# fakerlove1/HPFG

Hardware: AMD Instinct MI355X
Metric: labeled+unlabeled images/sec/node, U-Net 224x224 ACDC-shaped (Mean-Teacher step) (higher is better)
Workload: dtype bf16x3 (fp32 storage; products as split-bf16 MFMA hi*hi+hi*lo+lo*hi, fp32 accumulate); 1 GPU; mean_teacher_unet_224x224 (BASELINE configs[1]): U-Net 1ch->4cls, 8 labelled + 8 unlabelled per GPU, student fwd+bwd + train-mode teacher fwd + CE/Dice/MSE + SGD + EMA; size=224, hipgraph=True, sync_bn=False, parallelism=dp1, math=bf16x3

## Files before the change

hpfg_amd/_lib.py:

```python
from __future__ import annotations

import ctypes as C
import os
import threading

_HERE = os.path.dirname(os.path.abspath(__file__))
LIB_PATH = os.path.join(_HERE, "lib", "libhpfg_hip.so")

BN_MEAN, BN_RSTD, BN_SCALE, BN_SHIFT, BN_K1, BN_K2, BN_K3, BN_SPARE, BN_ROWS = range(9)
ACT_NONE, ACT_PLAIN, ACT_STRIDED, ACT_BNACT, ACT_BNACT_POOL, ACT_UP2X, ACT_DZ, ACT_SPLIT16, ACT_UPBWD = range(9)
OPT_CONV_THIN, OPT_FIRST_MFMA, OPT_FIRST_WGRAD, OPT_NARROW_DEEP = 0, 1, 2, 3
LOSS_NSUM = 32
LOSS_MAX_CLASSES = 16
ACC_MAX_SHARDS = 8
VERSION = 136
RESIZE_TAPS = 36
MATH_F32, MATH_BF16X3 = 0, 1


class HipLibraryError(RuntimeError):
    pass


class Act(C.Structure):
    _fields_ = [("z", C.c_void_p), ("bn", C.c_void_p), ("aux", C.c_void_p), ("mode", C.c_int32), ("C", C.c_int32),
                ("Hs", C.c_int32), ("Ws", C.c_int32), ("pstride", C.c_int32), ("aux_pstride", C.c_int32),
                ("bn_stride", C.c_int32), ("bn_coff", C.c_int32), ("sn", C.c_int32), ("sc", C.c_int32), ("sy", C.c_int32),
                ("sx", C.c_int32), ("drop_p", C.c_float), ("drop_seed", C.c_uint32), ("drop_mask", C.c_void_p), ("seed_dev", C.c_void_p),
                ("bn_acc", C.c_void_p), ("bn_gamma", C.c_void_p), ("bn_beta", C.c_void_p), ("bn_count", C.c_float), ("bn_eps", C.c_float),
                ("bn_shards", C.c_int32), ("reserved1", C.c_int32)]


class ConvArgs(C.Structure):
    _fields_ = [("a0", Act), ("a1", Act), ("wpk", C.c_void_p), ("bias", C.c_void_p), ("out", C.c_void_p),
                ("stat_partials", C.c_void_p), ("out_pstride", C.c_int32), ("Cout", C.c_int32), ("CoutPad", C.c_int32),
                ("N", C.c_int32), ("H", C.c_int32), ("W", C.c_int32), ("taps", C.c_int32), ("math", C.c_int32),
                ("bwd_stats", C.c_int32), ("bwd_of", Act), ("out2", C.c_void_p), ("out_split", C.c_int32), ("out2_pstride", C.c_int32),
                ("stat_acc", C.c_void_p), ("stat_shards", C.c_int32), ("reserved2", C.c_int32), ("stage_out", C.c_void_p), ("side_sums", C.c_void_p)]


class WgradArgs(C.Structure):
    _fields_ = [("a0", Act), ("a1", Act), ("g", Act), ("slab", C.c_void_p), ("dw_oihw", C.c_void_p), ("Cin", C.c_int32),
                ("CinPad", C.c_int32), ("Cout", C.c_int32), ("CoutPad", C.c_int32), ("N", C.c_int32), ("H", C.c_int32),
                ("W", C.c_int32), ("taps", C.c_int32), ("S", C.c_int32), ("math", C.c_int32), ("defer_reduce", C.c_int32)]


class PeerX(C.Structure):
    _fields_ = [("mbox", C.c_void_p * 8), ("epoch", C.c_void_p), ("err", C.c_void_p), ("world", C.c_int32), ("rank", C.c_int32),
                ("slot", C.c_int32), ("cap", C.c_int32), ("slot_bytes", C.c_int64)]


class PeerBuf(C.Structure):
    _fields_ = [("win", C.c_void_p * 8), ("epoch", C.c_void_p), ("err", C.c_void_p), ("world", C.c_int32), ("rank", C.c_int32),
                ("slice", C.c_int64), ("n", C.c_int64), ("stride", C.c_int64)]


class FusedBwdArgs(C.Structure):
    _fields_ = [("d", ConvArgs), ("xa0", Act), ("xa1", Act), ("slab", C.c_void_p), ("Cin", C.c_int32), ("CinPad", C.c_int32),
                ("Cout", C.c_int32), ("CoutPad", C.c_int32)]


class AugSample(C.Structure):
    _fields_ = [("img_off", C.c_int64), ("lab_off", C.c_int64), ("h", C.c_int32), ("w", C.c_int32), ("mode", C.c_int32), ("k", C.c_int32),
                ("axis", C.c_int32), ("tab_off", C.c_int32), ("m00", C.c_double), ("m01", C.c_double), ("m10", C.c_double),
                ("m11", C.c_double), ("off_y", C.c_double), ("off_x", C.c_double)]


class BnAccDesc(C.Structure):
    _fields_ = [("acc", C.c_void_p), ("gamma", C.c_void_p), ("beta", C.c_void_p), ("running_mean", C.c_void_p), ("running_var", C.c_void_p),
                ("bn", C.c_void_p), ("C", C.c_int32), ("count", C.c_float), ("shards", C.c_int32), ("reserved", C.c_int32)]


class BnAccBwdDesc(C.Structure):
    _fields_ = [("acc", C.c_void_p), ("gamma", C.c_void_p), ("bn", C.c_void_p), ("dgamma", C.c_void_p), ("dbeta", C.c_void_p),
                ("C", C.c_int32), ("count", C.c_float), ("shards", C.c_int32), ("reserved", C.c_int32)]


class SlabDesc(C.Structure):
    _fields_ = [("slab", C.c_void_p), ("dw_oihw", C.c_void_p), ("S", C.c_int32), ("taps", C.c_int32), ("Cin", C.c_int32),
                ("CinPad", C.c_int32), ("Cout", C.c_int32), ("CoutPad", C.c_int32)]


class PackDesc(C.Structure):
    _fields_ = [("w_oihw", C.c_void_p), ("b", C.c_void_p), ("wpk_fwd", C.c_void_p), ("wpk_dgrad", C.c_void_p),
                ("bias_pad", C.c_void_p), ("wpk16_fwd", C.c_void_p), ("wpk16_dgrad", C.c_void_p), ("Cout", C.c_int32), ("Cin", C.c_int32),
                ("CoutPad", C.c_int32), ("CinPad", C.c_int32), ("taps", C.c_int32), ("kc", C.c_int32)]


class LossArgs(C.Structure):
    _fields_ = [("logits", C.c_void_p), ("t_logits", C.c_void_p), ("labels0", C.c_void_p), ("labels1", C.c_void_p),
                ("coef", C.c_void_p), ("partials", C.c_void_p), ("sums", C.c_void_p), ("out", C.c_void_p),
                ("dlogits", C.c_void_p), ("N", C.c_int32), ("n_lab", C.c_int32), ("H", C.c_int32), ("W", C.c_int32),
                ("C", C.c_int32), ("world", C.c_int32), ("input_is_prob", C.c_int32), ("teacher_is_prob", C.c_int32),
                ("t_unlab_only", C.c_int32), ("reserved0", C.c_int32), ("cons_mask", C.c_void_p)]


class PredBlocks(C.Structure):
    _fields_ = [("p", C.c_void_p * 8), ("n_blocks", C.c_int32), ("per_block", C.c_int32)]
# ... 75 lines not shown
    "hpfg_linear_wgrad": (_i, [_p, _p, _p, _p, _l, _i, _i, _p]),
    "hpfg_linear_wgrad_splits": (_i, [_l, _i, _i]),
    "hpfg_tok_col_stats": (_i, [_p, _l, _i, _p, _p, _p]),
    "hpfg_tok_stat_blocks": (_i, [_l]),
    "hpfg_bnrelu_apply": (_i, [_p, _p, _p, _p, _p, _p, _f, _l, _p, _l, _i, _p]),
    "hpfg_bnrelu_bwd": (_i, [_p, _p, _p, _p, _p, _p, _p, _f, _l, _p, _p, _p, _l, _i, _p]),
    "hpfg_noise_add": (_i, [_p, _p, _p, _l, _l, _f, _f, _f, _p]),
    "hpfg_uncertainty_mask": (_i, [C.POINTER(PredBlocks), _i, _i, _i, _i, _i, _p, _p, _p, _p]),
    "hpfg_mix_samples": (_i, [_p, _p, _p, _p, _i, _l, _p]),
    "hpfg_softmax_mix": (_i, [_p, _p, _p, _p, _i, _i, _i, _i, _p]),
    "hpfg_pool_scatter_add": (_i, [C.POINTER(Act), _p, _i, _p, _i, _i, _i, _i, _p]),
    "hpfg_upsample2x_bwd": (_i, [_p, _i, _p, _i, _i, _i, _i, _p]),
    "hpfg_upsample2x_bwd_sums": (_i, [_p, _i, _p, _i, _i, _i, _i, _p, _p]),
    "hpfg_upsample2x_bwd_blocks": (_i, [_i, _i, _i, _i]),
    "hpfg_loss_blocks": (_i, [_i, _i, _i]),
    "hpfg_loss_nsum": (_i, [_i]),
    "hpfg_seg_loss_partials": (_i, [C.POINTER(LossArgs), _p]),
    "hpfg_seg_loss_finalize": (_i, [C.POINTER(LossArgs), _p]),
    "hpfg_seg_loss_bwd": (_i, [C.POINTER(LossArgs), _p, _p]),
    "hpfg_argmax_labels": (_i, [_p, _i, _i, _i, _i, _p, _p, _p, _p]),
    "hpfg_cutmix_blend": (_i, [_p, _p, _p, _p, _l, _p]),
    "hpfg_sgd_step": (_i, [_p, _p, _p, _l, _p, _f, _f, _f, _p]),
    "hpfg_adamw_step": (_i, [_p, _p, _p, _p, _l, _p, _p, _f, _f, _f, _f, _f, _p]),
    "hpfg_ema_update": (_i, [_p, _p, _l, _p, _p]),
    "hpfg_sgd_ema_step": (_i, [_p, _p, _p, _l, _p, _f, _f, _f, _p, _l, _p, _p]),
    "hpfg_attn_mfma_fwd": (_i, [_p, _p, _p, _i, _i, _i, _i, _f, _p]),
    "hpfg_attn_mfma_bwd": (_i, [_p, _p, _p, _p, _p, _p, _i, _i, _i, _i, _f, _p]),
    "hpfg_attn_mfma_blocks": (_i, [_i]),
    "hpfg_attn_mfma_fwd_hd": (_i, [_p, _p, _p, _i, _i, _i, _i, _i, _f, _p]),
    "hpfg_attn_mfma_bwd_hd": (_i, [_p, _p, _p, _p, _p, _p, _i, _i, _i, _i, _i, _f, _p]),
    "hpfg_attn_mfma_scratch_floats": (_l, [_i, _i, _i, _i]),
    "hpfg_attn_keys_max": (_i, []),
    "hpfg_attn_keys_fwd": (_i, [_p, _p, _p, _p, _i, _i, _i, _i, _i, _f, _i, _p]),
    "hpfg_attn_keys_bwd": (_i, [_p, _p, _p, _p, _p, _p, _p, _p, _i, _i, _i, _i, _i, _f, _i, _p]),
    "hpfg_attn_keys_scratch_floats": (_l, [_i, _i, _i, _i, _i, _i]),
    "hpfg_attn_fwd_hd": (_i, [_p, _p, _p, _i, _i, _i, _i, _i, _f, _p]),
    "hpfg_attn_bwd_hd": (_i, [_p, _p, _p, _p, _p, _p, _i, _i, _i, _i, _i, _f, _p]),
    "hpfg_gemm_f32": (_i, [_p, _l, _l, _p, _l, _l, _p, _l, _i, _i, _i, _p, _i, _i, _p]),
    "hpfg_gemm_f32_splitk": (_i, [_p, _l, _l, _p, _l, _l, _p, _l, _i, _i, _i, _p, _i, _i, _p, _p]),
    "hpfg_gemm_f32_splits": (_i, [_i, _i, _i]),
    "hpfg_gemm_bf16x3": (_i, [_p, _l, _l, _p, _l, _l, _p, _l, _i, _i, _i, _p, _i, _i, _p]),
    "hpfg_gemm_bf16x3_splits": (_i, [_i, _i, _i]),
    "hpfg_gemm_bf16x3_splitk": (_i, [_p, _l, _l, _p, _l, _l, _p, _l, _i, _i, _i, _p, _i, _i, _p, _p]),
    "hpfg_gemm_bf16x3_ok": (_i, [_p, _l, _l, _p, _l, _l, _i, _i, _i]),
    "hpfg_gemm_tn_bf16x3": (_i, [_p, _p, _p, _p, _l, _i, _i, _i, _p]),
    "hpfg_gemm_tn_splits": (_i, [_l, _i, _i]),
    "hpfg_col_sum2": (_i, [_p, _l, _i, _l, _p, _p, _p]),
    "hpfg_col_sum_splits": (_i, [_l]),
    "hpfg_col_sum": (_i, [_p, _l, _i, _l, _p, _p]),
    "hpfg_relu_bwd": (_i, [_p, _p, _l, _p]),
    "hpfg_neck_pool_fwd": (_i, [_p, _i, _i, _i, _i, _i, _i, _p, _p, _p]),
    "hpfg_neck_pool_bwd": (_i, [_p, _p, _i, _i, _i, _i, _i, _p, _p]),
    "hpfg_l2norm_fwd": (_i, [_p, _i, _i, _i, _i, _i, _p, _p, _p]),
    "hpfg_l2norm_bwd": (_i, [_p, _p, _p, _i, _i, _i, _i, _i, _p, _p, _p]),
    "hpfg_ntxent_rows": (_i, [_p, _i, _f, _p, _p, _p]),
}

_lock = threading.Lock()
_lib = None


def load() -> C.CDLL:
    global _lib
    if _lib is not None:
        return _lib
    with _lock:
        if _lib is not None:
            return _lib
        if not os.path.exists(LIB_PATH):
            raise HipLibraryError(
                f"{LIB_PATH} not found: build it with `python -c 'import __graft_entry__ as g; g.build()'` "
                f"or `make -C hpfg_amd/csrc`. There is no CPU fallback for the HIP path.")
        lib = C.CDLL(LIB_PATH)
        for name, (res, args) in PROTOTYPES.items():
            fn = getattr(lib, name)
            fn.restype = res
            fn.argtypes = args
        if lib.hpfg_version() != VERSION:
            raise HipLibraryError(f"libhpfg_hip.so version {lib.hpfg_version()} != binding version {VERSION}; rebuild")
        if os.environ.get("HPFG_FIRST_WGRAD", "1") == "0":
            lib.hpfg_set_option(OPT_FIRST_WGRAD, 0)
        if os.environ.get("HPFG_NARROW_DEEP") is not None:
            lib.hpfg_set_option(OPT_NARROW_DEEP, int(os.environ["HPFG_NARROW_DEEP"]))
        _lib = lib
    return _lib


def check(rc: int, what: str):
    if rc != 0:
        msg = load().hpfg_last_error().decode("utf-8", "replace")
        raise HipLibraryError(f"{what} failed (rc={rc}): {msg}")


def ptr(t):
    return None if t is None else t.data_ptr()


def none_act() -> Act:
    return Act()
```

hpfg_amd/csrc/conv_bf16_kernel.h:

```cpp
#pragma once
#include <stdlib.h>
#include "stage.h"

namespace hpfg_conv16 {

using namespace hpfg_stage;

template <int TH_, int TW_, int WM_, int WN_, int NI_, int TAPS_, int KC_>
struct Cfg {
  static constexpr int TH = TH_, TW = TW_, WM = WM_, WN = WN_, NI = NI_, TAPS = TAPS_, KC = KC_;
  static constexpr int MI = TH * TW / 16 / WM;
  static constexpr int BN = 16 * NI * WN;
  static constexpr int HALO = TAPS == 9 ? 1 : 0;
  static constexpr int HP = TH + 2 * HALO, WP = TW + 2 * HALO;
  static constexpr int RS = TW == 16 ? WP : (TAPS == 9 ? 24 : 8);
  static constexpr int NSLOT = (HP * RS + 15) / 16 * 16;
  static constexpr int NG = KC / 8;
  static constexpr int PLANE = NSLOT * 16;
  static constexpr int BUF_BYTES = NG * 2 * PLANE;
  static constexpr int KSTEPS = TAPS == 1 ? 1 : (KC == 32 ? 9 : 5);
  static constexpr int NPIECE = HP * WP * NG;
  static constexpr int NLD = (NPIECE + 255) / 256;
  static_assert(WM * WN == 4, "4 waves per workgroup");
  static_assert(256 % NG == 0, "a thread must keep one channel group");
// ... 93 lines not shown
    for (int m = 0; m < C::MI; ++m) {
      const int pxl = (wm * C::MI + m) * 16 + (lane & 15);
      const int gy = ty0 + pxl / C::TW, gx = tx0 + pxl % C::TW;
      if (pool) {
        if (gy < H && gx < W && co < p.Cout) {
          const f32x4 v = acc[m][j];
          float* dA = const_cast<float*>(p.bwd_of.aux);
          const long p00 = ((long)n * p.bwd_of.Hs + 2 * gy) * p.bwd_of.Ws + 2 * gx;
          f32x4 z4[4], g4[4];
#pragma unroll
          for (int k = 0; k < 4; ++k) {
            const long off = p00 + (k >> 1) * p.bwd_of.Ws + (k & 1);
            z4[k] = *reinterpret_cast<const f32x4*>(p.bwd_of.z + off * p.bwd_of.pstride + co);
            g4[k] = *reinterpret_cast<const f32x4*>(dA + off * p.bwd_of.aux_pstride + co);
          }
#pragma unroll
          for (int r = 0; r < 4; ++r) {
            float y[4];
#pragma unroll
            for (int k = 0; k < 4; ++k) y[k] = z4[k][r] * tsc[r] + tsh[r];
            float best = lrelu(y[0]);
            int bi = 0;
#pragma unroll
            for (int k = 1; k < 4; ++k) {
              const float a = lrelu(y[k]);
              if (a > best) {
                best = a;
                bi = k;
              }
            }
#pragma unroll
            for (int k = 0; k < 4; ++k) {
              g4[k][r] += bi == k ? v[r] : 0.f;
              const float gg = y[k] > 0.f ? g4[k][r] : HPFG_LEAKY * g4[k][r];
              s1[j][r] += gg;
              s2[j][r] += gg * z4[k][r];
            }
          }
#pragma unroll
          for (int k = 0; k < 4; ++k) {
            const long off = p00 + (k >> 1) * p.bwd_of.Ws + (k & 1);
            *reinterpret_cast<f32x4*>(dA + off * p.bwd_of.aux_pstride + co) = g4[k];
          }
        }
        continue;
      }
      if (gy < H && gx < W && co < p.Cout) {
        f32x4 v = acc[m][j] + b;
        float* o = (p.out_split && co >= p.out_split) ? p.out2 + ((n * H + gy) * W + gx) * p.out2_pstride + (co - p.out_split)
                                                       : p.out + ((n * H + gy) * W + gx) * p.out_pstride + co;
        if (p.math & 0x100) {
        } else if (vec) {
          *reinterpret_cast<f32x4*>(o) = v;
        } else {
#pragma unroll
          for (int r = 0; r < 4; ++r) {
            if (co + r < p.Cout) o[r] = v[r];
            else v[r] = 0.f;
          }
        }
        if (bwd) {
          const long pix = ((long)n * H + gy) * W + gx;
          const f32x4 z = zq[m];
          uint32_t km = 0xFu;
          if (p.bwd_of.drop_p > 0.f) km = keep4(p.bwd_of, bcx, (uint32_t)(pix * p.bwd_of.C + co));
#pragma unroll
          for (int r = 0; r < 4; ++r) {
            float gg = (km >> r) & 1u ? v[r] * bcx.inv_keep : 0.f;
            gg = z[r] * tsc[r] + tsh[r] > 0.f ? gg : HPFG_LEAKY * gg;
            s1[j][r] += gg;
            s2[j][r] += gg * z[r];
          }
        } else {
          s1[j] += v;
          s2[j] += v * v;
        }
      }
    }
  }
}

template <class C, int BWD = 0>
__device__ __forceinline__ void conv16_flush_stats(const HpfgConvArgs& p, f32x4 (&s1)[C::NI], f32x4 (&s2)[C::NI], float* ldsf, int tid, int lane, int wm,
                                                   int wn, int cb, int row) {
  if ((!p.stat_partials && !p.stat_acc) || (p.math & 0x1000)) return;
#pragma unroll
  for (int j = 0; j < C::NI; ++j)
#pragma unroll
    for (int r = 0; r < 4; ++r) {
      float a = s1[j][r], b = s2[j][r];
#pragma unroll
      for (int o = 1; o < 16; o <<= 1) {
        a += __shfl_xor(a, o);
        b += __shfl_xor(b, o);
      }
      s1[j][r] = a;
      s2[j][r] = b;
    }
  if ((lane & 15) == 0) {
#pragma unroll
    for (int j = 0; j < C::NI; ++j) {
      const int cl = (wn * C::NI + j) * 16 + (lane >> 4) * 4;
      *reinterpret_cast<f32x4*>(ldsf + (0 * C::WM + wm) * C::BN + cl) = s1[j];
      *reinterpret_cast<f32x4*>(ldsf + (1 * C::WM + wm) * C::BN + cl) = s2[j];
    }
  }
  __syncthreads();
  if (tid < 2 * C::BN) {
    const int which = tid / C::BN, cl = tid % C::BN;
    float t = 0.f;
#pragma unroll
    for (int w = 0; w < C::WM; ++w) t += ldsf[(which * C::WM + w) * C::BN + cl];
    const int co = cb * C::BN + cl;
    if (BWD && p.bwd_stats && which == 1 && co < p.Cout) {
      float sg = 0.f;
#pragma unroll
      for (int w = 0; w < C::WM; ++w) sg += ldsf[w * C::BN + cl];
      const float* tb = p.bwd_of.bn + p.bwd_of.bn_coff + co;
      t = tb[HPFG_BN_RSTD * p.bwd_of.bn_stride] * (t - tb[HPFG_BN_MEAN * p.bwd_of.bn_stride] * sg);
    }
    if (p.stat_acc && co < p.Cout)
      hpfg_acc_add(p.stat_acc, p.CoutPad, ((int)blockIdx.z * (int)gridDim.y + (int)blockIdx.y) * (int)gridDim.x + (int)blockIdx.x & (p.stat_shards - 1), which, co, t);
    if (p.stat_partials && co < p.CoutPad) p.stat_partials[((long)row * 2 + which) * p.CoutPad + co] = t;
  }
}

#define HPFG16_MFMA3(ACC, AH, AL, BH, BL)                              \
  ACC = __builtin_amdgcn_mfma_f32_16x16x32_bf16(BH, AH, ACC, 0, 0, 0); \
  ACC = __builtin_amdgcn_mfma_f32_16x16x32_bf16(BL, AH, ACC, 0, 0, 0); \
  ACC = __builtin_amdgcn_mfma_f32_16x16x32_bf16(BH, AL, ACC, 0, 0, 0);

template <class C>
struct UpGeo {
  static constexpr int SH = C::TH / 2 + 3, SW = C::TW / 2 + 3;
  static constexpr int NPIECE = SH * SW * C::NG;
  static constexpr int BYTES = SH * SW * C::KC * 4;
  static_assert(NPIECE <= 256, "one source piece per thread");
};
template <int KIND>
constexpr int eff_nr() { return KIND == HPFG_KIND_CAT ? 2 : RawCount<KIND>::N; }

__device__ __forceinline__ int up_base(int o0, int L) {
  const float r = L > 1 ? (float)(L - 1) / (float)(2 * L - 1) : 0.f;
  return (int)(r * (float)(o0 < 0 ? 0 : o0));
}

template <class C, int KIND>
constexpr int wg_per_cu() {
  return (C::KSTEPS == 5 && C::NI == 1 && RawCount<KIND>::N <= 2) ? 3 : 2;
}

#ifdef HPFG_TRACE
#define HPFG_TR(ID)                                                                                        \
  if (tr_on && tr_i < 255) {                                                                               \
    tr_buf[tr_i++] = ((unsigned long long)(ID) << 56) | (__builtin_amdgcn_s_memtime() & 0xffffffffffffffull); \
  }
#define HPFG_TR_REAL(ID)                                                                                   \
  if (tr_on && tr_i < 255) {                                                                               \
    tr_buf[tr_i++] = ((unsigned long long)(ID) << 56) | (__builtin_amdgcn_s_memrealtime() & 0xffffffffffffffull); \
  }
#else
#define HPFG_TR(ID)
#define HPFG_TR_REAL(ID)
#endif

template <class C, int KIND, int BWD = 0>
__global__ __launch_bounds__(256, (wg_per_cu<C, KIND>())) void conv_bf16x3_kernel(HpfgConvArgs p, int tiles_x, int tiles_y) {
  static_assert(C::TAPS == 9, "persistent kernel is the 3x3 path");
  constexpr int STAT_BYTES = 2 * 4 * C::BN * 4;
  constexpr int NR = eff_nr<KIND>();
  constexpr bool CATK = KIND == HPFG_KIND_CAT;
  constexpr int UP_BYTES = CATK ? UpGeo<C>::BYTES : 0;
  __shared__ __attribute__((aligned(16))) unsigned char lds[2 * C::BUF_BYTES + STAT_BYTES + UP_BYTES];
  float* ldsf = reinterpret_cast<float*>(lds + 2 * C::BUF_BYTES);
  float* ldsU = reinterpret_cast<float*>(lds + 2 * C::BUF_BYTES + STAT_BYTES);
  (void)ldsU;
  constexpr bool TABK = tab_in_lds<KIND>();
  __shared__ __attribute__((aligned(16))) float ldsBN[TABK ? tab_rows<KIND>() * HPFG_BN_CMAX : 4];
  (void)ldsBN;
  const int tid = threadIdx.x, lane = tid & 63, wave = tid >> 6;
  const int wm = wave % C::WM, wn = wave / C::WM;
  const int cb = blockIdx.y;
  const int H = p.H, W = p.W;
  const int ntiles = tiles_x * tiles_y, nwork = ntiles * p.N;
  const ActCtx cx0 = make_ctx(p.a0);
  constexpr bool SIDE = KIND != HPFG_KIND_PLAIN && C::TH == 4;
  const bool dzw = SIDE && p.stage_out != nullptr && cb == 0;
  (void)dzw;
#ifdef HPFG_TRACE
  const bool tr_on = (p.math & 0x2000) && tid == 0;
  unsigned long long* tr_buf = reinterpret_cast<unsigned long long*>(p.stat_partials) + 256 * ((long)blockIdx.y * gridDim.x + blockIdx.x);
  int tr_i = 0;
#endif
  HPFG_TR_REAL(11)
  HPFG_TR(1)

  f32x4 acc[C::MI][C::NI];
#pragma unroll
  for (int m = 0; m < C::MI; ++m)
#pragma unroll
    for (int j = 0; j < C::NI; ++j) acc[m][j] = f32x4{0.f, 0.f, 0.f, 0.f};

  const int kg = lane >> 4;
  const int gl = C::KC == 32 ? kg : (kg & 1);
  int aoff[C::MI];
// ... 348 lines not shown
        f32x4 v[2] = {f32x4{0.f, 0.f, 0.f, 0.f}, f32x4{0.f, 0.f, 0.f, 0.f}};
#pragma unroll
        for (int hq = 0; hq < 2; ++hq) {
          f32x4 t[HPFG_UPB_TAPS][HPFG_UPB_TAPS];
#pragma unroll
          for (int a = 0; a < HPFG_UPB_TAPS; ++a) {
            const float* row = src + (long)upI[q.ly][a] * Wo * ps + 4 * hq;
#pragma unroll
            for (int b = 0; b < HPFG_UPB_TAPS; ++b) t[a][b] = *reinterpret_cast<const f32x4*>(row + ix[b]);
          }
          f32x4 acc = {0.f, 0.f, 0.f, 0.f};
#pragma unroll
          for (int a = 0; a < HPFG_UPB_TAPS; ++a) {
            f32x4 h = wx[0] * t[a][0];
#pragma unroll
            for (int b = 1; b < HPFG_UPB_TAPS; ++b) h += wx[b] * t[a][b];
            acc += hpfg_own_vgpr(upW[q.ly][a]) * h;
          }
#pragma unroll
          for (int j = 0; j < 4; ++j) v[hq][j] = ok ? acc[j] : 0.f;
        }
        store_piece<C, HPFG_KIND_PLAIN>(lds, q, v[0], v[1]);
        if (side && ok) {
          if (p.stage_out) {
            float* d = p.stage_out + ((long)(n * H + gy) * W + gx) * p.a0.C + c0c;
            *reinterpret_cast<f32x4*>(d) = v[0];
            *reinterpret_cast<f32x4*>(d + 4) = v[1];
          }
          cs0 += v[0];
          cs1 += v[1];
        }
      }
      if (side && p.side_sums) {
        *reinterpret_cast<f32x4*>(upS + tid * 8) = cs0;
        *reinterpret_cast<f32x4*>(upS + tid * 8 + 4) = cs1;
      }
    } else {
#pragma unroll
    for (int i = 0; i < C::NLD; ++i) {
      const Piece q = make_piece<C>(tid, i);
      const int gy = ty0 + q.ly, gx = tx0 + q.lx;
      const bool ok = q.ok && chv && gy < H && gx < W;
      RawPiece<KIND> raw;
      f32x4 v0, v1;
      const int gyc = clampi(gy, 0, H - 1), gxc = clampi(gx, 0, W - 1), c0c = chv ? c0 : 0;
      issue_piece<KIND>(raw, p.a0, p.a1, cx0, n, gyc, gxc, c0c, ok);
      finish_piece<KIND>(v0, v1, raw, tab, p.a0, p.a1, cx0, n, gyc, gxc, c0c, ok);
      store_piece<C, KIND>(lds, q, v0, v1);
    }
    }
    bf16x8 bh[C::NI], bl[C::NI];
    load_b<C>(bh, bl, wpk, ch, ntn, nt0, lane);
    __syncthreads();
    if constexpr (UPB) {
      if (side && p.side_sums && tid < C::KC) {
        const int g = tid >> 3, j = tid & 7;
        float tsum = 0.f;
        for (int k = g; k < 256; k += C::NG) tsum += upS[k * 8 + j];
        const int cch = ch * C::KC + tid;
        if (cch < p.a0.C) p.side_sums[(long)wg_row * p.a0.C + cch] = tsum;
      }
    }
#pragma unroll
    for (int m = 0; m < C::MI; ++m) {
      const bf16x8 ah = *reinterpret_cast<const bf16x8*>(lds + aoff[m]);
      const bf16x8 al = *reinterpret_cast<const bf16x8*>(lds + aoff[m] + C::PLANE);
#pragma unroll
      for (int j = 0; j < C::NI; ++j) { HPFG16_MFMA3(acc[m][j], ah, al, bh[j], bl[j]) }
    }
  }
  f32x4 s1[C::NI], s2[C::NI];
#pragma unroll
  for (int j = 0; j < C::NI; ++j) {
    s1[j] = f32x4{0.f, 0.f, 0.f, 0.f};
    s2[j] = s1[j];
  }
  f32x4 bias[C::NI];
  conv16_load_bias<C>(p, bias, lane, nt0);
  conv16_store_tile<C, BWD>(p, acc, s1, s2, bias, lane, wm, nt0, n, ty0, tx0);
  __syncthreads();
  conv16_flush_stats<C, BWD>(p, s1, s2, ldsf, tid, lane, wm, wn, cb, n * (tiles_x * tiles_y) + tile);
}

template <class C, int KIND>
int persistent_grid(const HpfgConvArgs& a) {
  const int tx = (a.W + C::TW - 1) / C::TW, ty = (a.H + C::TH - 1) / C::TH;
  const int lds_bytes = 2 * C::BUF_BYTES + 2 * 4 * C::BN * 4;
  int per_cu = 160 * 1024 / lds_bytes;
  const int reg_cap = wg_per_cu<C, KIND>();
  if (per_cu > reg_cap) per_cu = reg_cap;
  if (per_cu < 1) per_cu = 1;
  const long nwork = (long)tx * ty * a.N;
  const long gy = a.CoutPad / C::BN;
  long cap = 256L * per_cu / (gy > 0 ? gy : 1);
  if (cap < 1) cap = 1;
  const long rounds = (nwork + cap - 1) / cap;
  return (int)((nwork + rounds - 1) / rounds);
}

template <class C, int KIND>
int launch_cfg(const HpfgConvArgs& a, hipStream_t st, int* rows_only) {
  int tx = (a.W + C::TW - 1) / C::TW, ty = (a.H + C::TH - 1) / C::TH;
  if (rows_only) {
    if constexpr (C::TAPS == 9) *rows_only = persistent_grid<C, KIND>(a);
    else *rows_only = tx * ty * a.N;
    return 0;
  }
  if constexpr (C::TAPS == 9) {
    dim3 grid((unsigned)persistent_grid<C, KIND>(a), a.CoutPad / C::BN);
    if (a.stat_acc) HPFG_ACC_CHECK((long)grid.x * grid.y, a.stat_shards, "conv_fwd");
    if constexpr (KIND == HPFG_KIND_DZ || KIND == HPFG_KIND_PLAIN) {
      if constexpr (C::TH == 4) {
        if (a.bwd_stats == 2) {
          hipLaunchKernelGGL((conv_bf16x3_kernel<C, KIND, 2>), grid, dim3(256), 0, st, a, tx, ty);
          return hpfg_launch_status("conv_bf16x3_kernel<bwd stats + pool>");
        }
      }
      if (a.bwd_stats == 2) {
        hpfg_set_error("conv_fwd: bwd_stats == 2 is built for H or W not a multiple of 16");
        return -1;
      }
      if (a.bwd_stats) {
        hipLaunchKernelGGL((conv_bf16x3_kernel<C, KIND, 1>), grid, dim3(256), 0, st, a, tx, ty);
        return hpfg_launch_status("conv_bf16x3_kernel<bwd stats>");
      }
    }
    hipLaunchKernelGGL((conv_bf16x3_kernel<C, KIND>), grid, dim3(256), 0, st, a, tx, ty);
  } else {
    dim3 grid(tx * ty, a.N, a.CoutPad / C::BN);
    if (a.stat_acc) HPFG_ACC_CHECK((long)grid.x * grid.y * grid.z, a.stat_shards, "conv_fwd(1x1)");
    if constexpr (KIND == HPFG_KIND_DZ || KIND == HPFG_KIND_PLAIN || KIND == HPFG_KIND_UPB) {
      if (a.bwd_stats) {
        hipLaunchKernelGGL((conv1x1_bf16x3_kernel<C, KIND, 1>), grid, dim3(256), 0, st, a, tx, ty);
        return hpfg_launch_status("conv1x1_bf16x3_kernel<bwd stats>");
      }
    }
    hipLaunchKernelGGL((conv1x1_bf16x3_kernel<C, KIND>), grid, dim3(256), 0, st, a, tx, ty);
  }
  return hpfg_launch_status("conv_bf16x3_kernel");
}

template <int KIND, int TAPS>
int conv_dispatch_kind(const HpfgConvArgs& a, hipStream_t st, int* rows_only) {
  const bool big = (a.H % 16 == 0) && (a.W % 16 == 0);
  const int cp = a.CoutPad;
  constexpr int KCB = TAPS == 9 ? 16 : 32;
  if (big) {
    if constexpr (TAPS == 1) {
      if (cp % 64 == 0) return launch_cfg<Cfg<16, 16, 4, 1, 4, TAPS, KCB>, KIND>(a, st, rows_only);
    }
    if (cp % 32 == 0) return launch_cfg<Cfg<16, 16, 4, 1, 2, TAPS, KCB>, KIND>(a, st, rows_only);
    return launch_cfg<Cfg<16, 16, 4, 1, 1, TAPS, KCB>, KIND>(a, st, rows_only);
  }
  if constexpr (TAPS == 9) {
    {
      const long tiles = (long)a.N * ((a.H + 3) / 4) * ((a.W + 15) / 16);
      if (cp % 64 == 0 && tiles * (cp / 64) <= hpfg_opt(HPFG_OPT_NARROW_DEEP))
        return launch_cfg<Cfg<4, 16, 2, 2, 1, TAPS, 32>, KIND>(a, st, rows_only);
    }
    if (cp % 64 == 0) return launch_cfg<Cfg<4, 16, 1, 4, 1, TAPS, 32>, KIND>(a, st, rows_only);
    if (cp % 32 == 0) return launch_cfg<Cfg<4, 16, 2, 2, 1, TAPS, 32>, KIND>(a, st, rows_only);
    return launch_cfg<Cfg<4, 16, 4, 1, 1, TAPS, 32>, KIND>(a, st, rows_only);
  }
  const long nwork = (long)a.N * ((a.H + 7) / 8) * ((a.W + 7) / 8);
  if (cp % 128 == 0 && nwork * (cp / 128) >= 512) return launch_cfg<Cfg<8, 8, 1, 4, 2, TAPS, 32>, KIND>(a, st, rows_only);
  if (cp % 64 == 0 && (nwork * (cp / 64) >= 512 || cp % 32 != 0)) return launch_cfg<Cfg<8, 8, 1, 4, 1, TAPS, 32>, KIND>(a, st, rows_only);
  if (cp % 32 == 0) return launch_cfg<Cfg<8, 8, 2, 2, 1, TAPS, 32>, KIND>(a, st, rows_only);
  return launch_cfg<Cfg<8, 8, 4, 1, 1, TAPS, 32>, KIND>(a, st, rows_only);
}

}

constexpr int HPFG_THIN_NONE = -100;
int hpfg_conv_thin_try(const HpfgConvArgs& a, hipStream_t st, int* rows_only);
int hpfg_conv16_launch_plain(const HpfgConvArgs& a, hipStream_t st, int* rows_only);
int hpfg_conv16_launch_bnact(const HpfgConvArgs& a, hipStream_t st, int* rows_only);
int hpfg_conv16_launch_pool(const HpfgConvArgs& a, hipStream_t st, int* rows_only);
int hpfg_conv16_launch_cat(const HpfgConvArgs& a, hipStream_t st, int* rows_only);
int hpfg_conv16_launch_dz(const HpfgConvArgs& a, hipStream_t st, int* rows_only);
int hpfg_conv16_launch_upb(const HpfgConvArgs& a, hipStream_t st, int* rows_only);
```

hpfg_amd/csrc/misc.hip:

```cpp
#include <stdarg.h>
#include <string.h>
#include "stage.h"

static thread_local char g_err[512] = "";
extern "C" void hpfg_set_error(const char* fmt, ...) {
  va_list ap;
  va_start(ap, fmt);
  vsnprintf(g_err, sizeof(g_err), fmt, ap);
  va_end(ap);
}
extern "C" const char* hpfg_last_error(void) { return g_err; }
extern "C" int hpfg_version(void) { return HPFG_VERSION; }

static int g_opt[HPFG_OPT_COUNT] = {1, 1, 1, 128};
int hpfg_opt(int which) { return which >= 0 && which < HPFG_OPT_COUNT ? g_opt[which] : 0; }
extern "C" int hpfg_set_option(int which, int value) {
  HPFG_ARG_CHECK(which >= 0 && which < HPFG_OPT_COUNT, "set_option: unknown option %d", which);
  const int old = g_opt[which];
  g_opt[which] = value;
  return old;
}

namespace {

__global__ __launch_bounds__(256) void pack_weights_kernel(const HpfgPackDesc* __restrict__ table, long long* __restrict__ counters, int n_counters,
                                                           int* __restrict__ seed_word, int seed_add, long long* __restrict__ zero, long n_zero) {
  if (blockIdx.x == 0 && blockIdx.y == 0) {
    for (int i = threadIdx.x; i < n_counters; i += 256) counters[i] += 1;
    if (threadIdx.x == 0 && seed_word && seed_add) *seed_word = (*seed_word + seed_add) & 0x7FFFFFFF;
  }
  for (long i = ((long)blockIdx.y * gridDim.x + blockIdx.x) * 256 + threadIdx.x; i < n_zero; i += (long)gridDim.x * gridDim.y * 256) zero[i] = 0;
  const HpfgPackDesc d = table[blockIdx.y];
  const long total = (long)d.taps * d.CinPad * d.CoutPad;
  const int nt_f = d.CoutPad / 16, nch_f = d.CinPad / 16;
  const int nt_d = d.CinPad / 16, nch_d = d.CoutPad / 16;
  for (long i = blockIdx.x * 256L + threadIdx.x; i < total; i += (long)gridDim.x * 256) {
    int ks = (int)(i & 3), lane = (int)((i >> 2) & 63);
    long r = i >> 8;
    if (d.wpk_fwd) {
      int nt = (int)(r % nt_f), ch = (int)((r / nt_f) % nch_f), tap = (int)(r / ((long)nt_f * nch_f));
      int co = nt * 16 + (lane & 15), ci = ch * 16 + ks * 4 + (lane >> 4);
      d.wpk_fwd[i] = (co < d.Cout && ci < d.Cin) ? d.w_oihw[((long)co * d.Cin + ci) * d.taps + tap] : 0.f;
    }
    if (d.wpk_dgrad) {
      int nt = (int)(r % nt_d), ch = (int)((r / nt_d) % nch_d), tap = (int)(r / ((long)nt_d * nch_d));
      int co = ch * 16 + ks * 4 + (lane >> 4), ci = nt * 16 + (lane & 15);
      d.wpk_dgrad[i] = (co < d.Cout && ci < d.Cin) ? d.w_oihw[((long)co * d.Cin + ci) * d.taps + (d.taps - 1 - tap)] : 0.f;
    }
    if (i < d.CoutPad) d.bias_pad[i] = (i < d.Cout && d.b) ? d.b[i] : 0.f;
  }
  const int ksteps = d.taps == 1 ? 1 : (d.kc == 32 ? 9 : 5);
  for (int dir = 0; dir < 2; ++dir) {
    __bf16* out = reinterpret_cast<__bf16*>(dir == 0 ? d.wpk16_fwd : d.wpk16_dgrad);
    if (!out) continue;
    const int Kch = dir == 0 ? d.Cin : d.Cout;
    const int ntn = (dir == 0 ? d.CoutPad : d.CinPad) / 16;
    const int nchunks = (Kch + d.kc - 1) / d.kc;
    const long tot = (long)nchunks * ksteps * ntn * 512;
    for (long i = blockIdx.x * 256L + threadIdx.x; i < tot; i += (long)gridDim.x * 256) {
      const int j = (int)(i & 7), lane = (int)((i >> 3) & 63);
      const long r = i >> 9;
      const int nt = (int)(r % ntn), ks = (int)(r / ntn);
      const int chunk = ks / ksteps, s = ks % ksteps;
      const int kl = 8 * (lane >> 4) + j;
      int tap, kch;
      if (d.taps == 1) { tap = 0; kch = chunk * 32 + kl; }
      else if (d.kc == 32) { tap = s; kch = chunk * 32 + kl; }
      else { tap = 2 * s + (kl >> 4); kch = chunk * 16 + (kl & 15); }
      const int nch = nt * 16 + (lane & 15);
      float w = 0.f;
      if (tap < d.taps && kch < Kch) {
        if (dir == 0) { if (nch < d.Cout) w = d.w_oihw[((long)nch * d.Cin + kch) * d.taps + tap]; }
        else { if (nch < d.Cin) w = d.w_oihw[((long)kch * d.Cin + nch) * d.taps + (d.taps - 1 - tap)]; }
      }
      const __bf16 hi = (__bf16)w;
      const __bf16 lo = (__bf16)(w - (float)hi);
      const long base = ((long)ks * ntn + nt) * 2;
      out[(base + 0) * 512 + lane * 8 + j] = hi;
      out[(base + 1) * 512 + lane * 8 + j] = lo;
    }
  }
}

__global__ __launch_bounds__(256) void materialize_kernel(HpfgAct a0, HpfgAct a1, int N, int H, int W, float* __restrict__ out) {
  const int Ct = a0.C + a1.C, Q = (Ct + 3) / 4;
  const ActCtx c0 = make_ctx(a0), c1 = make_ctx(a1);
  const long total = (long)N * H * W * Q;
  for (long i = blockIdx.x * 256L + threadIdx.x; i < total; i += (long)gridDim.x * 256) {
    int q = (int)(i % Q);
    long pix = i / Q;
    int x = (int)(pix % W), y = (int)((pix / W) % H), n = (int)(pix / ((long)W * H));
    f32x4 v = cat_load4(a0, c0, a1, c1, n, y, x, q * 4);
#pragma unroll
    for (int j = 0; j < 4; ++j)
      if (q * 4 + j < Ct) out[pix * Ct + q * 4 + j] = v[j];
  }
}
// ... 535 lines not shown
```

include/hpfg_hip.h:

```cpp
#ifndef HPFG_HIP_H
#define HPFG_HIP_H

#include <stdint.h>

#ifdef __cplusplus
extern "C" {
#endif

#define HPFG_VERSION 136
enum { HPFG_MATH_F32 = 0, HPFG_MATH_BF16X3 = 1 };

enum { HPFG_BN_MEAN = 0, HPFG_BN_RSTD = 1, HPFG_BN_SCALE = 2, HPFG_BN_SHIFT = 3,
       HPFG_BN_K1 = 4, HPFG_BN_K2 = 5, HPFG_BN_K3 = 6, HPFG_BN_SPARE = 7, HPFG_BN_ROWS = 8 };

enum {
  HPFG_ACT_NONE = 0,
  HPFG_ACT_PLAIN = 1,
  HPFG_ACT_STRIDED = 2,
  HPFG_ACT_BNACT = 3,
  HPFG_ACT_BNACT_POOL = 4,
  HPFG_ACT_UP2X = 5,
  HPFG_ACT_DZ = 6,
  HPFG_ACT_SPLIT16 = 7,
  HPFG_ACT_UPBWD = 8
};

typedef struct HpfgAct {
  const float* z;
  const float* bn;
  const float* aux;
  int32_t mode;
  int32_t C;
  int32_t Hs, Ws;
  int32_t pstride;
  int32_t aux_pstride;
  int32_t bn_stride;
  int32_t bn_coff;
  int32_t sn, sc, sy, sx;
  float drop_p;
  uint32_t drop_seed;
  const uint8_t* drop_mask;
  const uint32_t* seed_dev;
  const long long* bn_acc;
  const float* bn_gamma;
  const float* bn_beta;
  float bn_count;
  float bn_eps;
  int32_t bn_shards;
  int32_t reserved1;
} HpfgAct;

typedef struct HpfgConvArgs {
  HpfgAct a0, a1;
  const float* wpk;
  const float* bias;
  float* out;
  float* stat_partials;
  int32_t out_pstride, Cout, CoutPad;
  int32_t N, H, W;
  int32_t taps;
  int32_t math;
  int32_t bwd_stats;
  HpfgAct bwd_of;
  float* out2;
  int32_t out_split;
  int32_t out2_pstride;
  long long* stat_acc;
  int32_t stat_shards;
  int32_t reserved2;
  float* stage_out;
  float* side_sums;
} HpfgConvArgs;
#define HPFG_ACC_MAX_SHARDS 8
#define HPFG_ACC_WORDS(C, shards) ((shards) * 2 * 2 * (C))

typedef struct HpfgWgradArgs {
  HpfgAct a0, a1;
  HpfgAct g;
  float* slab;
  float* dw_oihw;
  int32_t Cin, CinPad, Cout, CoutPad;
  int32_t N, H, W, taps;
  int32_t S;
  int32_t math;
  int32_t defer_reduce;
} HpfgWgradArgs;

typedef struct HpfgFusedBwdArgs {
  HpfgConvArgs d;
  HpfgAct xa0, xa1;
  float* slab;
  int32_t Cin, CinPad, Cout, CoutPad;
} HpfgFusedBwdArgs;

typedef struct HpfgSlabDesc {
  const float* slab;
  float* dw_oihw;
  int32_t S, taps, Cin, CinPad, Cout, CoutPad;
} HpfgSlabDesc;

typedef struct HpfgPackDesc {
  const float* w_oihw;
  const float* b;
  float* wpk_fwd;
  float* wpk_dgrad;
  float* bias_pad;
  void* wpk16_fwd;
  void* wpk16_dgrad;
  int32_t Cout, Cin, CoutPad, CinPad, taps;
  int32_t kc;
} HpfgPackDesc;

int hpfg_version(void);
const char* hpfg_last_error(void);
enum { HPFG_OPT_CONV_THIN = 0, HPFG_OPT_FIRST_MFMA = 1, HPFG_OPT_FIRST_WGRAD = 2, HPFG_OPT_NARROW_DEEP = 3, HPFG_OPT_COUNT = 4 };
int hpfg_set_option(int which, int value);

int hpfg_conv3x3_first_fwd(const HpfgAct* x, const float* w_oihw, const float* bias, float* out, float* stat_partials,
                           int N, int H, int W, int Cin, int Cout, void* stream);
int hpfg_conv_first_rows(int N, int H, int W);
int hpfg_conv3x3_first_fwd_acc(const HpfgAct* x, const float* w_oihw, const float* bias, float* out, float* stat_partials, long long* stat_acc,
                               int stat_shards, int N, int H, int W, int Cin, int Cout, void* stream);
int hpfg_conv_fwd(const HpfgConvArgs* args, void* stream);
int hpfg_conv_stat_blocks(int N, int H, int W);
int hpfg_conv_stat_rows(const HpfgConvArgs* args);
int hpfg_bn_fwd_finalize(const float* partials, int nblk, const double* sums, double count, const float* gamma, const float* beta,
                         float* running_mean, float* running_var, float momentum, float eps, float* bn, int C, void* stream);
typedef struct HpfgBnAccDesc {
  const long long* acc;
  const float* gamma;
  const float* beta;
  float* running_mean;
  float* running_var;
  float* bn;
  int32_t C;
  float count;
  int32_t shards;
  int32_t reserved;
} HpfgBnAccDesc;
int hpfg_bn_acc_finalize(const HpfgBnAccDesc* table_dev, const HpfgBnAccDesc* table_host, int nlayers, float momentum, float eps, void* stream);
typedef struct HpfgBnAccBwdDesc {
  long long* acc;
  const float* gamma;
  float* bn;
  float* dgamma;
  float* dbeta;
  int32_t C;
  float count;
  int32_t shards;
  int32_t reserved;
} HpfgBnAccBwdDesc;
int hpfg_bn_acc_bwd_finalize(const HpfgBnAccBwdDesc* table_dev, const HpfgBnAccBwdDesc* table_host, int nlayers, void* stream);
int hpfg_bn_bwd_reduce_acc(const HpfgAct* g, int N, int H, int W, long long* acc, int shards, void* stream);
int hpfg_bn_bwd_reduce_pool_acc(const HpfgAct* g, const float* dP, int dp_pstride, int N, int Hp, int Wp, long long* acc, int shards, void* stream);
int hpfg_reduce_partials(const float* partials, int nblk, int C, double* sums, void* stream);
int hpfg_bn_eval_table(const float* gamma, const float* beta, const float* running_mean, const float* running_var, float eps,
                       float* bn, int C, void* stream);
int hpfg_conv_kc(int H, int W, int taps);
long hpfg_wpk16_elems(int Kchannels, int NchannelsPad, int taps, int kc);
int hpfg_pack_weights(const HpfgPackDesc* table_dev, const HpfgPackDesc* table_host, int nlayers, void* stream);
int hpfg_pack_weights_bump(const HpfgPackDesc* table_dev, const HpfgPackDesc* table_host, int nlayers, long long* counters, int n_counters,
                           int32_t* seed_word, int seed_add, long long* zero_words, long n_zero, void* stream);
int hpfg_act_materialize(const HpfgAct* a0, const HpfgAct* a1, int N, int H, int W, float* out, void* stream);
int hpfg_dropout_mask(uint8_t* out, long n_elems, float p, uint32_t seed, const uint32_t* seed_dev, void* stream);

int hpfg_bn_bwd_reduce(const HpfgAct* g , int N, int H, int W, float* partials, void* stream);
int hpfg_bn_bwd_blocks(int N, int H, int W, int C);
int hpfg_bn_bwd_reduce_pool(const HpfgAct* g , const float* dP, int dp_pstride, int N, int Hp, int Wp,
                            float* partials , void* stream);
int hpfg_bn_bwd_pool_blocks(int N, int Hp, int Wp, int C);
int hpfg_bn_bwd_finalize(const float* partials, int nblk, const double* sums, double count, const float* gamma,
                         float* bn, float* dgamma, float* dbeta, int C, float param_grad_scale, void* stream);
int hpfg_wgrad(const HpfgWgradArgs* args, void* stream);
int hpfg_fused_bwd(const HpfgFusedBwdArgs* args, void* stream);
int hpfg_fused_bwd_grid(const HpfgFusedBwdArgs* args);
int hpfg_slab_reduce_multi(const HpfgSlabDesc* table_dev, const HpfgSlabDesc* table_host, int nlayers, void* stream);
int hpfg_wgrad_splits(int N, int H, int W, int CinPad, int CoutPad, int taps);
long hpfg_wgrad_slab_floats(int N, int H, int W, int CinPad, int CoutPad, int taps);
int hpfg_channel_sum(const float* g, int pstride, long npix, int C, float* out, float* scratch, void* stream);
int hpfg_channel_sum_partials(const float* g, int pstride, long npix, int C, float* partials, void* stream);
int hpfg_channel_sum_blocks(long npix, int C);
int hpfg_pool_scatter_add(const HpfgAct* src , const float* dP, int dp_pstride,
                          float* dA, int da_pstride, int N, int Hp, int Wp, void* stream);
int hpfg_upsample2x_bwd(const float* dUp, int dup_pstride, float* dU, int N, int Hl, int Wl, int C, void* stream);
int hpfg_upsample2x_bwd_sums(const float* dUp, int dup_pstride, float* dU, int N, int Hl, int Wl, int C, float* csum_partials, void* stream);
int hpfg_upsample2x_bwd_blocks(int N, int Hl, int Wl, int C);

#define HPFG_PEER_MAX_RANKS 8
#define HPFG_PEER_HANDLE_BYTES 64
#define HPFG_PEER_MAX_SPINS (1L << 22)
typedef struct HpfgPeerX {
  void* mbox[HPFG_PEER_MAX_RANKS];
  const int32_t* epoch;
  int32_t* err;
  int32_t world, rank;
  int32_t slot, cap;
  int64_t slot_bytes;
} HpfgPeerX;
// ... 168 lines not shown
```

Measured before the change: 7862 images/s.

## Add persistent streamed 1x1 conv kernel with prefetch across work items

Adds a persistent 1x1 bf16x3 conv kernel. Each workgroup walks several tile/channel-chunk work items and prefetches the next chunk's raw activation pieces into registers while computing the current one, using double-buffered LDS. Its grid is sized to a per-CU occupancy target, and BN stat accumulation uses a virtual workgroup index so shard selection stays consistent. It is enabled by default only for TH==8 configs, with an env option to force or cap it. This targets launch-tail and load-latency costs of the one-tile-per-block 1x1 kernel, at the cost of register pressure and less parallelism on small layers.

```diff
diff --git a/hpfg_amd/_lib.py b/hpfg_amd/_lib.py
--- a/hpfg_amd/_lib.py
+++ b/hpfg_amd/_lib.py
@@ -9,11 +9,11 @@
 
 BN_MEAN, BN_RSTD, BN_SCALE, BN_SHIFT, BN_K1, BN_K2, BN_K3, BN_SPARE, BN_ROWS = range(9)
 ACT_NONE, ACT_PLAIN, ACT_STRIDED, ACT_BNACT, ACT_BNACT_POOL, ACT_UP2X, ACT_DZ, ACT_SPLIT16, ACT_UPBWD = range(9)
-OPT_CONV_THIN, OPT_FIRST_MFMA, OPT_FIRST_WGRAD, OPT_NARROW_DEEP = 0, 1, 2, 3
+OPT_CONV_THIN, OPT_FIRST_MFMA, OPT_FIRST_WGRAD, OPT_NARROW_DEEP, OPT_CONV1X1_STREAM = 0, 1, 2, 3, 4
 LOSS_NSUM = 32
 LOSS_MAX_CLASSES = 16
 ACC_MAX_SHARDS = 8
-VERSION = 136
+VERSION = 137
 RESIZE_TAPS = 36
 MATH_F32, MATH_BF16X3 = 0, 1
 
@@ -255,6 +255,8 @@
             lib.hpfg_set_option(OPT_FIRST_WGRAD, 0)
         if os.environ.get("HPFG_NARROW_DEEP") is not None:
             lib.hpfg_set_option(OPT_NARROW_DEEP, int(os.environ["HPFG_NARROW_DEEP"]))
+        if os.environ.get("HPFG_CONV1X1_STREAM") is not None:
+            lib.hpfg_set_option(OPT_CONV1X1_STREAM, int(os.environ["HPFG_CONV1X1_STREAM"]))
         _lib = lib
     return _lib
 
diff --git a/hpfg_amd/csrc/conv_bf16_kernel.h b/hpfg_amd/csrc/conv_bf16_kernel.h
--- a/hpfg_amd/csrc/conv_bf16_kernel.h
+++ b/hpfg_amd/csrc/conv_bf16_kernel.h
@@ -199,7 +199,7 @@
 
 template <class C, int BWD = 0>
 __device__ __forceinline__ void conv16_flush_stats(const HpfgConvArgs& p, f32x4 (&s1)[C::NI], f32x4 (&s2)[C::NI], float* ldsf, int tid, int lane, int wm,
-                                                   int wn, int cb, int row) {
+                                                   int wn, int cb, int row, int vwg = -1) {
   if ((!p.stat_partials && !p.stat_acc) || (p.math & 0x1000)) return;
 #pragma unroll
   for (int j = 0; j < C::NI; ++j)
@@ -237,7 +237,7 @@
       t = tb[HPFG_BN_RSTD * p.bwd_of.bn_stride] * (t - tb[HPFG_BN_MEAN * p.bwd_of.bn_stride] * sg);
     }
     if (p.stat_acc && co < p.Cout)
-      hpfg_acc_add(p.stat_acc, p.CoutPad, ((int)blockIdx.z * (int)gridDim.y + (int)blockIdx.y) * (int)gridDim.x + (int)blockIdx.x & (p.stat_shards - 1), which, co, t);
+      hpfg_acc_add(p.stat_acc, p.CoutPad, (vwg >= 0 ? vwg : ((int)blockIdx.z * (int)gridDim.y + (int)blockIdx.y) * (int)gridDim.x + (int)blockIdx.x) & (p.stat_shards - 1), which, co, t);
     if (p.stat_partials && co < p.CoutPad) p.stat_partials[((long)row * 2 + which) * p.CoutPad + co] = t;
   }
 }
@@ -752,6 +752,193 @@
   conv16_flush_stats<C, BWD>(p, s1, s2, ldsf, tid, lane, wm, wn, cb, n * (tiles_x * tiles_y) + tile);
 }
 
+template <class C>
+struct StreamLds {
+  static constexpr int PAIR = 4 * C::PLANE + 64;
+  static constexpr int BUF = 2 * PAIR;
+  __device__ static __forceinline__ int off(int g, int slot) { return (g >> 1) * PAIR + (g & 1) * 2 * C::PLANE + ((slot ^ ((g & 1) << 1)) * 16); }
+};
+template <class C, int KIND>
+constexpr int stream_depth() { return C::NLD == 1 ? (C::NI >= 2 ? 2 : 4) : 1; }
+template <class C>
+constexpr int stream_wg_per_cu() { return C::TH == 8 ? 3 : 2; }
+template <class C>
+constexpr int stream_grid_per_cu() { return C::TH == 8 ? 4 : 2; }
+
+struct StreamCur {
+  int w, n, tyi, txi, ch;
+};
+
+template <class C, int KIND, int BWD = 0>
+__global__ __launch_bounds__(256, (stream_wg_per_cu<C>())) void conv1x1_stream_kernel(HpfgConvArgs p, int tiles_x, int tiles_y) {
+  static_assert(C::TAPS == 1 && C::KC == 32 && KIND != HPFG_KIND_UPB, "streamed 1x1 path");
+  static_assert(C::NPIECE == C::NLD * 256, "every thread stages NLD pieces");
+  using L = StreamLds<C>;
+  constexpr int D = stream_depth<C, KIND>();
+  constexpr int STAT_BYTES = 2 * 4 * C::BN * 4;
+  __shared__ __attribute__((aligned(16))) unsigned char lds[2 * L::BUF + STAT_BYTES];
+  float* ldsf = reinterpret_cast<float*>(lds + 2 * L::BUF);
+  constexpr bool TABK = tab_in_lds<KIND>();
+  __shared__ __attribute__((aligned(16))) float ldsBN[TABK ? tab_rows<KIND>() * HPFG_BN_CMAX : 4];
+  (void)ldsBN;
+  const int tid = threadIdx.x, lane = tid & 63, wave = tid >> 6;
+  const int wm = wave % C::WM, wn = wave / C::WM;
+  const int cb = blockIdx.y;
+  const int H = p.H, W = p.W;
+  const int ntiles = tiles_x * tiles_y, nwork = ntiles * p.N;
+  const ActCtx cx0 = make_ctx(p.a0);
+
+  const int nx = gridDim.x >= 8 ? 8 : 1;
+  const int xg = (int)blockIdx.x % nx, xj = (int)blockIdx.x / nx;
+  const int per_x = (nwork + nx - 1) / nx;
+  const int wend = (xg + 1) * per_x < nwork ? (xg + 1) * per_x : nwork;
+  const int G = ((int)gridDim.x - xg + nx - 1) / nx;
+  const int w0 = xg * per_x + xj;
+  if (w0 >= wend) return;
+  const int gn = G / ntiles, gty = (G % ntiles) / tiles_x, gtx = (G % ntiles) % tiles_x;
+  auto next_group = [&](StreamCur c, int nchunks) {
+    c.ch += D;
+    if (c.ch < nchunks) return c;
+    c.ch = 0;
+    c.w += G;
+    c.txi += gtx;
+    c.tyi += gty;
+    c.n += gn;
+    if (c.txi >= tiles_x) {
+      c.txi -= tiles_x;
+      ++c.tyi;
+    }
+    if (c.tyi >= tiles_y) {
+      c.tyi -= tiles_y;
+      ++c.n;
+    }
+    return c;
+  };
+
+  const int g4 = tid % C::NG, g8 = g4 * 8;
+  int ply[C::NLD], plx[C::NLD], plds[C::NLD];
+#pragma unroll
+  for (int i = 0; i < C::NLD; ++i) {
+    const int pix = (tid + i * 256) / C::NG;
+    ply[i] = pix / C::TW;
+    plx[i] = pix % C::TW;
+    plds[i] = L::off(g4, ply[i] * C::RS + plx[i]);
+  }
+  const int kg = lane >> 4;
+  int aoff[C::MI];
+#pragma unroll
+  for (int m = 0; m < C::MI; ++m) {
+    const int pxl = (wm * C::MI + m) * 16 + (lane & 15);
+    aoff[m] = L::off(kg, (pxl / C::TW) * C::RS + (pxl % C::TW));
+  }
+  const int cin_total = p.a0.C + p.a1.C;
+  const int nchunks = (cin_total + C::KC - 1) / C::KC;
+  const int ntn = p.CoutPad / 16;
+  const int nt0 = (cb * C::WN + wn) * C::NI;
+  const bf16x8* wpk = reinterpret_cast<const bf16x8*>(p.wpk);
+
+  auto issue = [&](RawPiece<KIND> (&raw)[C::NLD], const StreamCur& c, int d) {
+    const int c0 = (c.ch + d) * C::KC + g8;
+    const bool chv = c0 < cin_total;
+    const int c0c = chv ? c0 : 0;
+#pragma unroll
+    for (int i = 0; i < C::NLD; ++i) {
+      const int gy = c.tyi * C::TH + ply[i], gx = c.txi * C::TW + plx[i];
+      const bool ok = chv && gy < H && gx < W;
+      issue_piece<KIND>(raw[i], p.a0, p.a1, cx0, c.n, clampi(gy, 0, H - 1), clampi(gx, 0, W - 1), c0c, ok);
+    }
+  };
+
+  StreamCur cur = {w0, w0 / ntiles, (w0 % ntiles) / tiles_x, (w0 % ntiles) % tiles_x, 0};
+  RawPiece<KIND> raw[D][C::NLD];
+#pragma unroll
+  for (int d = 0; d < D; ++d)
+    if (d < nchunks) issue(raw[d], cur, d);
+  f32x4 bias[C::NI];
+  conv16_load_bias<C>(p, bias, lane, nt0);
+  if constexpr (TABK) {
+    fill_tables_lds<KIND>(p.a0, ldsBN, tid, 256);
+    __syncthreads();
+  }
+  f32x4 acc[C::MI][C::NI];
+#pragma unroll
+  for (int m = 0; m < C::MI; ++m)
+#pragma unroll
+    for (int j = 0; j < C::NI; ++j) acc[m][j] = f32x4{0.f, 0.f, 0.f, 0.f};
+
+  int item = 0;
+  while (cur.w < wend) {
+    const StreamCur nxt = next_group(cur, nchunks);
+    const int ty0 = cur.tyi * C::TH, tx0 = cur.txi * C::TW;
+#pragma unroll
+    for (int d = 0; d < D; ++d) {
+      const bool pf = nxt.w < wend && nxt.ch + d < nchunks;
+      if (cur.ch + d < nchunks) {
+        unsigned char* buf = lds + (item & 1) * L::BUF;
+        ++item;
+        bf16x8 bh[C::NI], bl[C::NI];
+        load_b<C>(bh, bl, wpk, cur.ch + d, ntn, nt0, lane);
+        {
+          const int c0 = (cur.ch + d) * C::KC + g8;
+          const bool chv = c0 < cin_total;
+          const int c0c = chv ? c0 : 0;
+          Tab tab;
+          if constexpr (TABK) load_tables_lds<KIND>(tab, ldsBN, p.a0, c0c);
+          else load_tables<KIND>(tab, p.a0, c0, chv);
+#pragma unroll
+          for (int i = 0; i < C::NLD; ++i) {
+            const int gy = ty0 + ply[i], gx = tx0 + plx[i];
+            const bool ok = chv && gy < H && gx < W;
+            f32x4 v0, v1;
+            finish_piece<KIND>(v0, v1, raw[d][i], tab, p.a0, p.a1, cx0, cur.n, clampi(gy, 0, H - 1), clampi(gx, 0, W - 1), c0c, ok);
+            bf16x8 hi, lo;
+            split_piece<KIND>(v0, v1, hi, lo);
+            *reinterpret_cast<bf16x8*>(buf + plds[i]) = hi;
+            *reinterpret_cast<bf16x8*>(buf + plds[i] + C::PLANE) = lo;
+          }
+        }
+        if (pf) issue(raw[d], nxt, d);
+        __syncthreads();
+#pragma unroll
+        for (int m = 0; m < C::MI; ++m) {
+          const bf16x8 ah = *reinterpret_cast<const bf16x8*>(buf + aoff[m]);
+          const bf16x8 al = *reinterpret_cast<const bf16x8*>(buf + aoff[m] + C::PLANE);
+#pragma unroll
+          for (int j = 0; j < C::NI; ++j) { HPFG16_MFMA3(acc[m][j], ah, al, bh[j], bl[j]) }
+        }
+      } else if (pf) {
+        issue(raw[d], nxt, d);
+      }
+    }
+    if (cur.ch + D >= nchunks) {
+      f32x4 s1[C::NI], s2[C::NI];
+#pragma unroll
+      for (int j = 0; j < C::NI; ++j) {
+        s1[j] = f32x4{0.f, 0.f, 0.f, 0.f};
+        s2[j] = s1[j];
+      }
+      conv16_store_tile<C, BWD>(p, acc, s1, s2, bias, lane, wm, nt0, cur.n, ty0, tx0);
+      conv16_flush_stats<C, BWD>(p, s1, s2, ldsf, tid, lane, wm, wn, cb, cur.w, cb * nwork + cur.w);
+#pragma unroll
+      for (int m = 0; m < C::MI; ++m)
+#pragma unroll
+        for (int j = 0; j < C::NI; ++j) acc[m][j] = f32x4{0.f, 0.f, 0.f, 0.f};
+    }
+    cur = nxt;
+  }
+}
+
+template <class C>
+int stream_grid(long nwork, long slices) {
+  long cap = 256L * stream_grid_per_cu<C>() / (slices > 0 ? slices : 1);
+  if (cap < 1) cap = 1;
+  const long rounds = (nwork + cap - 1) / cap;
+  long g = (nwork + rounds - 1) / rounds;
+  const int v = hpfg_opt(HPFG_OPT_CONV1X1_STREAM);
+  if (v > 1 && g > v) g = v;
+  return (int)g;
+}
+
 template <class C, int KIND>
 int persistent_grid(const HpfgConvArgs& a) {
   const int tx = (a.W + C::TW - 1) / C::TW, ty = (a.H + C::TH - 1) / C::TH;
@@ -799,6 +986,20 @@
   } else {
     dim3 grid(tx * ty, a.N, a.CoutPad / C::BN);
     if (a.stat_acc) HPFG_ACC_CHECK((long)grid.x * grid.y * grid.z, a.stat_shards, "conv_fwd(1x1)");
+    if constexpr (KIND != HPFG_KIND_UPB) {
+      const int v = hpfg_opt(HPFG_OPT_CONV1X1_STREAM);
+      if (v > 1 || (v == 1 && C::TH == 8)) {
+        const dim3 sgrid((unsigned)stream_grid<C>((long)tx * ty * a.N, grid.z), grid.z);
+        if constexpr (KIND == HPFG_KIND_DZ || KIND == HPFG_KIND_PLAIN) {
+          if (a.bwd_stats) {
+            hipLaunchKernelGGL((conv1x1_stream_kernel<C, KIND, 1>), sgrid, dim3(256), 0, st, a, tx, ty);
+            return hpfg_launch_status("conv1x1_stream_kernel<bwd stats>");
+          }
+        }
+        hipLaunchKernelGGL((conv1x1_stream_kernel<C, KIND>), sgrid, dim3(256), 0, st, a, tx, ty);
+        return hpfg_launch_status("conv1x1_stream_kernel");
+      }
+    }
     if constexpr (KIND == HPFG_KIND_DZ || KIND == HPFG_KIND_PLAIN || KIND == HPFG_KIND_UPB) {
       if (a.bwd_stats) {
         hipLaunchKernelGGL((conv1x1_bf16x3_kernel<C, KIND, 1>), grid, dim3(256), 0, st, a, tx, ty);
diff --git a/hpfg_amd/csrc/misc.hip b/hpfg_amd/csrc/misc.hip
--- a/hpfg_amd/csrc/misc.hip
+++ b/hpfg_amd/csrc/misc.hip
@@ -12,7 +12,7 @@
 extern "C" const char* hpfg_last_error(void) { return g_err; }
 extern "C" int hpfg_version(void) { return HPFG_VERSION; }
 
-static int g_opt[HPFG_OPT_COUNT] = {1, 1, 1, 128};
+static int g_opt[HPFG_OPT_COUNT] = {1, 1, 1, 128, 1};
 int hpfg_opt(int which) { return which >= 0 && which < HPFG_OPT_COUNT ? g_opt[which] : 0; }
 extern "C" int hpfg_set_option(int which, int value) {
   HPFG_ARG_CHECK(which >= 0 && which < HPFG_OPT_COUNT, "set_option: unknown option %d", which);
diff --git a/include/hpfg_hip.h b/include/hpfg_hip.h
--- a/include/hpfg_hip.h
+++ b/include/hpfg_hip.h
@@ -7,7 +7,7 @@
 extern "C" {
 #endif
 
-#define HPFG_VERSION 136
+#define HPFG_VERSION 137
 enum { HPFG_MATH_F32 = 0, HPFG_MATH_BF16X3 = 1 };
 
 enum { HPFG_BN_MEAN = 0, HPFG_BN_RSTD = 1, HPFG_BN_SCALE = 2, HPFG_BN_SHIFT = 3,
@@ -113,7 +113,7 @@
 
 int hpfg_version(void);
 const char* hpfg_last_error(void);
-enum { HPFG_OPT_CONV_THIN = 0, HPFG_OPT_FIRST_MFMA = 1, HPFG_OPT_FIRST_WGRAD = 2, HPFG_OPT_NARROW_DEEP = 3, HPFG_OPT_COUNT = 4 };
+enum { HPFG_OPT_CONV_THIN = 0, HPFG_OPT_FIRST_MFMA = 1, HPFG_OPT_FIRST_WGRAD = 2, HPFG_OPT_NARROW_DEEP = 3, HPFG_OPT_CONV1X1_STREAM = 4, HPFG_OPT_COUNT = 5 };
 int hpfg_set_option(int which, int value);
 
 int hpfg_conv3x3_first_fwd(const HpfgAct* x, const float* w_oihw, const float* bias, float* out, float* stat_partials,
```

After: 7875 images/s, median of 6. About the same (+0.2%).
